# Alisah-Ozcan/HEonGPU

Hardware: AMD Instinct MI355X
Metric: homomorphic mults/sec (CKKS N=2^16, L=16) + NTT GB/s vs HBM roofline (higher is better)
Workload: dtype u64

## Files before the change

heongpu_amd/csrc/fpmod.cuh:

```cuda
#pragma once
#include "modarith.cuh"

namespace hegpu {

enum FpSiteKind {
    FPS_NONE = 0, FPS_FWD_COL = 1, FPS_FWD_COL_DECOMP = 2, FPS_FWD_ROW = 3, FPS_FWD_SINGLE = 4, FPS_KS_ROW = 5,
    FPS_KS_ROW_SPLIT = 6, FPS_INV = 7, FPS_TFHE_PREP = 8, FPS_TFHE_BR = 9, FPS_KINDS = 10
};
enum FpMetric { FPM_MUL_Y = 0, FPM_MUL_W = 1, FPM_MUL_T = 2, FPM_SUM = 3, FPM_RED_IN = 4, FPM_ABS = 5, FPM_COUNT = 6 };
#define FP_SITE(kind, sub) ((kind) * 8 + (sub))
#define FP_STAGE_PRODUCT 24
#define FP_STAGE_SUMS 25
#define FP_STAGE_INPUT 29
#define FP_STAGE_OUT 30
#define FP_STAGES 32

#ifdef HEGPU_FP_AUDIT_HEADER
#include HEGPU_FP_AUDIT_HEADER
#else
#define FP_AUDIT_FC_FIELDS
#define FP_AUDIT_INIT(c, site)
#define FP_STAGE(c, s)
#define FP_AUDIT_MUL(y, wx, wy, k, t, c)
#define FP_AUDIT_REDUCE(x, r, c)
#define FP_AUDIT_CANON(r, c)
#define FP_AUDIT_VAL(c, metric, v)
#define FP_AUDIT_FROM_U64(v)
#define FP_AUDIT_TO_U64(r)
#endif

struct FC {
    double q;
    double qi;
    FP_AUDIT_FC_FIELDS
};
__device__ __forceinline__ FC make_fc(u64 q, int site = FPS_NONE)
{
    FC c;
    c.q = (double) q;
    c.qi = 1.0 / c.q;
    FP_AUDIT_INIT(c, site);
    (void) site;
    return c;
}
__device__ __forceinline__ double as_f64(u64 v) { return __longlong_as_double((long long) v); }
__device__ __forceinline__ u64 as_bits(double v) { return (u64) __double_as_longlong(v); }
__device__ __forceinline__ double fp_from_u64(u64 v)
{
    FP_AUDIT_FROM_U64(v);
    return as_f64(v | 0x4330000000000000ull) - 4503599627370496.0;
}
__device__ __forceinline__ double fp_from_u32(u32 v) { return fp_from_u64((u64) v); }
__device__ __forceinline__ u64 fp_to_u64(double r)
{
    FP_AUDIT_TO_U64(r);
    return as_bits(r + 4503599627370496.0) & 0xFFFFFFFFFFFFFull;
}
__device__ __forceinline__ double fp_reduce(double x, const FC& c)
{
    const double r = __builtin_fma(-__builtin_rint(x * c.qi), c.q, x);
    FP_AUDIT_REDUCE(x, r, c);
    return r;
}
__device__ __forceinline__ double fp_canon(double x, const FC& c)
{
    const double r = fp_reduce(x, c);
    const double o = r < 0.0 ? r + c.q : r;
// ... 15 lines not shown
```

heongpu_amd/csrc/ntt.hip:

```cpp
#include "ntt.hpp"
#define HEGPU_FP_TU ntt
#include "fpmod.cuh"

namespace hegpu {

#define NTT_THREADS 256

#ifdef NTT_ABLATION_HEADER
#include NTT_ABLATION_HEADER
#else
__device__ __forceinline__ u64 gld(const u64* p) { return *p; }
__device__ __forceinline__ void gst(u64* p, u64 v) { *p = v; }
#define NTT_ABLATE_BFLY(x, y, w)
#define NTT_ABLATE_FPBFLY(x, y, w)
#define NTT_ABLATE_TW(load, root0, s) (load)
#define NTT_FP_TW(t, i, c) ((t)[i])
#endif

__device__ __forceinline__ u64 csub(u64 x, u64 m) { return (x >= m) ? x - m : x; }

typedef unsigned long long u64x2_t __attribute__((ext_vector_type(2)));
struct ConstTw {
    const u64x2_t __attribute__((address_space(4)))* p;
    __device__ __forceinline__ ulonglong2 operator[](u32 i) const
// ... 120 lines not shown
        const int half = 8 >> s;
        if (s > 0) __builtin_amdgcn_sched_barrier(0);
        if (s > 0) FP_STAGE(c, (c).stage + 1);
#pragma unroll
        for (int b = 0; b < (1 << s); b++) {
            const double wd = tb[((1 << s) - 1 + b) * 16];
            const ulonglong2 w = make_ulonglong2(as_bits(wd), as_bits(wd * c.qi));
#pragma unroll
            for (int j = 0; j < half; j++) fp_ct_bfly(x[b * 2 * half + j], x[b * 2 * half + j + half], w, c);
        }
    }
    FP_STAGE(c, (c).stage + 1);
#pragma unroll
    for (int k = 0; k < 16; k++) x[k] = fp_canon(x[k], c);
}

struct QC {
    u64 q;
    u64 q4;
    u32 nq0, nq1;
};
__device__ __forceinline__ QC make_qc(u64 q)
{
    QC c;
    c.q = q;
    c.q4 = 4 * q;
    u64 nq = 0 - q;
    c.nq0 = (u32) nq;
    c.nq1 = (u32) (nq >> 32);
    return c;
}

__device__ __forceinline__ u64 shoup_lazy(u64 y, ulonglong2 w, const QC& c)
{
    const u32 y0 = (u32) y, y1 = (u32) (y >> 32);
    const u32 w0 = (u32) w.x, w1 = (u32) (w.x >> 32), p0 = (u32) w.y, p1 = (u32) (w.y >> 32);
    const u64 A = (u64) y0 * p1;
    const u64 B = (u64) y1 * p0 + (u32) A;
    const u64 qh = (u64) y1 * p1 + (A >> 32) + (B >> 32);
    const u32 h0 = (u32) qh, h1 = (u32) (qh >> 32);
    u64 acc = (u64) y0 * w0;
    acc += (u64) h0 * c.nq0;
    const u32 hi = y0 * w1 + y1 * w0 + h0 * c.nq1 + h1 * c.nq0;
    return acc + ((u64) hi << 32);
}

__device__ __forceinline__ u64 shoup_full(u64 y, ulonglong2 w, const QC& c)
{
    u64 r = shoup_lazy(y, w, c);
    r = csub(r, 2 * c.q);
    return csub(r, c.q);
}

template <bool LAZY>
__device__ __forceinline__ void ct_bfly(u64& x, u64& y, ulonglong2 w, const QC& c)
{
    NTT_ABLATE_BFLY(x, y, w);
    u64 u = LAZY ? x : csub(x, c.q4);
    u64 t = shoup_lazy(y, w, c);
    x = u + t;
    y = u + c.q4 - t;
}

__device__ __forceinline__ void gs_bfly(u64& x, u64& y, ulonglong2 w, const QC& c)
{
    NTT_ABLATE_BFLY(x, y, w);
    u64 s = x + y;
    u64 d = x + c.q4 - y;
    x = csub(s, c.q4);
    y = shoup_lazy(d, w, c);
}

template <int LOGR, bool LAZY, typename TW>
__device__ __forceinline__ void ct_radix(u64 (&x)[1 << LOGR], TW tw,
                                         u32 root0, const QC& c)
{
#pragma unroll
    for (int s = 0; s < LOGR; s++) {
        const int half = (1 << LOGR) >> (s + 1);
#pragma unroll
        for (int b = 0; b < (1 << s); b++) {
            ulonglong2 w = NTT_ABLATE_TW(tw[(root0 << s) + b], root0, s);
#pragma unroll
            for (int j = 0; j < half; j++)
                ct_bfly<LAZY>(x[b * 2 * half + j], x[b * 2 * half + j + half], w, c);
        }
    }
}

template <bool LAZY>
__device__ __forceinline__ void ct_radix16_tb(u64 (&x)[16], const ulonglong2* __restrict__ tb, const QC& c)
{
#pragma unroll
    for (int s = 0; s < 4; s++) {
        const int half = 8 >> s;
#pragma unroll
        for (int b = 0; b < (1 << s); b++) {
            ulonglong2 w = tb[((1 << s) - 1 + b) * 16];
#pragma unroll
            for (int j = 0; j < half; j++)
                ct_bfly<LAZY>(x[b * 2 * half + j], x[b * 2 * half + j + half], w, c);
        }
    }
}

template <int LOGR>
__device__ __forceinline__ void gs_radix(u64 (&x)[1 << LOGR], const ulonglong2* __restrict__ tw,
                                         u32 root0, const QC& c)
{
#pragma unroll
    for (int s = LOGR - 1; s >= 0; s--) {
        const int half = (1 << LOGR) >> (s + 1);
#pragma unroll
        for (int b = 0; b < (1 << s); b++) {
            ulonglong2 w = NTT_ABLATE_TW(tw[(root0 << s) + b], root0, s);
#pragma unroll
            for (int j = 0; j < half; j++)
                gs_bfly(x[b * 2 * half + j], x[b * 2 * half + j + half], w, c);
        }
    }
}

__device__ __forceinline__ void gs_radix16_tb(u64 (&x)[16], const ulonglong2* __restrict__ tb, const QC& c)
{
#pragma unroll
    for (int s = 3; s >= 0; s--) {
        const int half = 8 >> s;
#pragma unroll
        for (int b = 0; b < (1 << s); b++) {
            ulonglong2 w = tb[((1 << s) - 1 + b) * 16];
#pragma unroll
            for (int j = 0; j < half; j++)
                gs_bfly(x[b * 2 * half + j], x[b * 2 * half + j + half], w, c);
        }
    }
}

template <int LOGR>
__device__ __forceinline__ void gs_radix_last(u64 (&x)[1 << LOGR], const ulonglong2* __restrict__ tw,
                                              u32 root0, ulonglong2 ninv, ulonglong2 w1ninv, const QC& c)
{
#pragma unroll
    for (int s = LOGR - 1; s >= 1; s--) {
        const int half = (1 << LOGR) >> (s + 1);
#pragma unroll
        for (int b = 0; b < (1 << s); b++) {
            ulonglong2 w = NTT_ABLATE_TW(tw[(root0 << s) + b], root0, s);
#pragma unroll
            for (int j = 0; j < half; j++)
                gs_bfly(x[b * 2 * half + j], x[b * 2 * half + j + half], w, c);
        }
    }
    const int half = (1 << LOGR) >> 1;
#pragma unroll
// ... 15 lines not shown
__device__ __forceinline__ int udiv16(int x, unsigned magic)
{
    return magic ? (int) __umulhi((unsigned) x, magic) : x;
}

__device__ __forceinline__ PolySel select_poly(const NttArgs& a, int poly)
{
    PolySel s;
    if (a.group_span) {
        const int k = udiv16(poly, a.mg_group_span), r = poly - k * a.group_span;
        if (a.polys_per_item) {
            const int per_item = udiv16(a.polys_per_item, a.mg_mod_count);
            const int it = udiv16(r, a.mg_per_item), d = r - it * per_item;
            poly = it * a.polys_per_item + d * a.mod_count + k;
        } else {
            poly = r * a.mod_count + k;
        }
    }
    int item = 0, j = poly;
    if (a.polys_per_item) {
        item = udiv16(poly, a.mg_polys_per_item);
        j = poly - item * a.polys_per_item;
    }
    int k = j - udiv16(j, a.mg_mod_count) * a.mod_count;
    if (a.mod_order) k = a.mod_order[k];
    s.mod = a.mod_offset + k;
    u64 slot = a.poly_order ? (u64) a.poly_order[j] : (u64) j;
    s.digit = a.decomp_mods ? udiv16(j, a.mg_decomp_mods) : -1;
    u64 in_slot = a.decomp_mods ? (u64) s.digit * (a.decomp_in_mul ? a.decomp_in_mul : 1) + a.decomp_in_add : slot;
    if (a.decomp_out_mul) slot = (u64) s.digit * a.decomp_out_mul + (u64) (j - s.digit * a.decomp_mods);
    s.in_off = (u64) item * a.in_item_stride + (in_slot << a.n_power);
    s.out_off = (u64) item * a.out_item_stride + (slot << a.n_power);
    s.item = item;
    s.j = j;
    return s;
}

__device__ __forceinline__ int col_phys(int e) { return e ^ (((e >> 8) & 1) << 4); }
__device__ __forceinline__ int row_phys(int e) { return e ^ (((e >> 5) & 7) << 1); }

__device__ __forceinline__ void wave_lds_fence()
{
    __builtin_amdgcn_fence(__ATOMIC_RELEASE, "wavefront");
    __builtin_amdgcn_wave_barrier();
    __builtin_amdgcn_fence(__ATOMIC_ACQUIRE, "wavefront");
}

#define COL_LDS_ELEMS 4096
#define ROW_LDS_ELEMS 4096

__device__ __forceinline__ bool fwd_stages_lazy(const Mod& md, u64 lazy_q_max) { return md.q <= lazy_q_max; }
#define NTT_ROW_LAZY_MAX_Q 0x0666666666666666ull
__device__ __forceinline__ bool row_stages_lazy(const Mod& md, u64 lazy_q_max) { return md.q <= lazy_q_max || md.q <= NTT_ROW_LAZY_MAX_Q; }

template <int S1, bool DECOMP, bool LAZY, bool SREG = false>
__device__ __forceinline__ void fwd_col_body(const NttArgs& a, const PolySel& ps, const Mod& md, u64* lds,
                                             const u64* sreg = nullptr)
{
    constexpr int R = 1 << S1;
    constexpr int CT = 4096 / R;
    constexpr int NSA = S1 - 4;
    constexpr int RA = 1 << NSA;
    constexpr int G = 16 / RA;
    const int t = threadIdx.x;
    const QC qc = make_qc(md.q);
    const ulonglong2* __restrict__ tw = a.tw + ((u64) ps.mod << a.n_power);
    const u64* __restrict__ src = a.in + ps.in_off + blockIdx.x * CT;
    u64* __restrict__ dst = a.out + ps.out_off + blockIdx.x * CT;

    const u64 half_qP = a.half_on ? a.mods[a.half_src_mod].q : 0;
    const u64 half_hm = a.half_on ? a.half_mod[ps.mod] : 0;
    u64 x[16];
    const int col = t % CT, r1 = t / CT;
    u64 v[16];
    if constexpr (NSA > 0) {
#pragma unroll
        for (int g = 0; g < G; g++) {
            const int L = t + NTT_THREADS * g;
            const int c = L % CT, rb = L / CT;
#pragma unroll
            for (int k = 0; k < RA; k++) v[g * RA + k] = SREG ? sreg[g * RA + k] : gld(&src[(u64) (rb + 16 * k) * 256 + c]);
        }
    } else {
#pragma unroll
        for (int k = 0; k < 16; k++) v[k] = SREG ? sreg[k] : gld(&src[(u64) k * 256 + col]);
    }
    if (DECOMP && a.half_on) {
#pragma unroll
        for (int k = 0; k < 16; k++) v[k] = sub_mod(reduce64(add_mod(v[k], a.half, half_qP), md), half_hm, md.q);
    } else if (DECOMP && !LAZY && a.mods[ps.digit].q > 8 * md.q) {
#pragma unroll
        for (int k = 0; k < 16; k++) v[k] = reduce64(v[k], md);
    }
    if constexpr (NSA > 0) {
#pragma unroll
        for (int g = 0; g < G; g++) {
            const int L = t + NTT_THREADS * g;
            const int c = L % CT, rb = L / CT;
            u64 y[RA];
#pragma unroll
            for (int k = 0; k < RA; k++) y[k] = v[g * RA + k];
            ct_radix<NSA, LAZY>(y, tw, 1u, qc);
#pragma unroll
            for (int k = 0; k < RA; k++) lds[col_phys((rb + 16 * k) * CT + c)] = y[k];
        }
        __syncthreads();
#pragma unroll
        for (int k = 0; k < 16; k++) x[k] = lds[col_phys((16 * r1 + k) * CT + col)];
        if (SREG) __syncthreads();
    } else {
#pragma unroll
        for (int k = 0; k < 16; k++) x[k] = v[k];
    }
    ct_radix<4, LAZY>(x, tw, (u32) (RA + r1), qc);
#pragma unroll
    for (int k = 0; k < 16; k++) gst(&dst[(u64) (16 * r1 + k) * 256 + col], x[k]);
}

template <int S1, bool DECOMP, bool WIDE, bool SREG = false>
__device__ __forceinline__ void fwd_col_body_fp(const NttArgs& a, const PolySel& ps, const Mod& md, u64* lds,
                                                ulonglong2* twl, const u64* sreg = nullptr)
{
    constexpr int R = 1 << S1;
    constexpr int CT = 4096 / R;
    constexpr int NSA = S1 - 4;
    constexpr int RA = 1 << NSA;
    constexpr int G = 16 / RA;
    const int t = threadIdx.x;
    const FC fc = make_fc(md.q, FP_SITE(DECOMP ? FPS_FWD_COL_DECOMP : FPS_FWD_COL, S1 - 4));
    const ulonglong2* __restrict__ tw = a.tw + ((u64) ps.mod << a.n_power);
    const u64* __restrict__ src = a.in + ps.in_off + blockIdx.x * CT;
    u64* __restrict__ dst = a.out + ps.out_off + blockIdx.x * CT;

    double c32 = 0.0, c32i = 0.0;
    if constexpr (DECOMP && WIDE) {
        c32 = (double) reduce64(1ull << 32, md);
        c32i = c32 * fc.qi;
    }
    const u64 half_qP = (DECOMP && a.half_on) ? a.mods[a.half_src_mod].q : 0;
    const double half_hm = (DECOMP && a.half_on) ? fp_from_u64(a.half_mod[ps.mod]) : 0.0;
    const bool in_small = S1 != 7 && DECOMP && !WIDE && !a.half_on && a.mods[ps.digit].q <= md.q + (md.q >> 6);
    typedef FpColSched<S1> CS;
    auto load_all = [&](auto& y, auto addr, int si0) {
        constexpr int CNT = sizeof(y) / sizeof(y[0]);
        FP_STAGE(fc, FP_STAGE_INPUT);
        if constexpr (SREG && !WIDE) {
            if (in_small) {
#pragma unroll
                for (int k = 0; k < CNT; k++) y[k] = as_f64(sreg[si0 + k]);
            } else {
#pragma unroll
                for (int k = 0; k < CNT; k++) y[k] = fp_reduce(as_f64(sreg[si0 + k]), fc);
            }
        } else {
            u64 v[CNT];
#pragma unroll
            for (int k = 0; k < CNT; k++) {
                v[k] = SREG ? sreg[si0 + k] : *addr(k);
                if constexpr (SREG) asm volatile("" : "+v"(v[k]));
            }
            if (!SREG && DECOMP && a.half_on) {
#pragma unroll
                for (int k = 0; k < CNT; k++) v[k] = add_mod(v[k], a.half, half_qP);
            }
#pragma unroll
            for (int k = 0; k < CNT; k++) {
                if constexpr (DECOMP && WIDE) y[k] = fp_mul(fp_from_u32((u32) (v[k] >> 32)), c32, c32i, fc) + fp_from_u32((u32) v[k]);
// ... 26 lines not shown
        }
        twl[t] = mine;
        __syncthreads();
#pragma unroll
        for (int k = 0; k < 16; k++) x[k] = as_f64(lds[col_phys((16 * r1 + k) * CT + col)]);
        if (SREG) __syncthreads();
        fp_ct_radix<4>(x, twl, (u32) (RA + r1), fc, CS::b_before, CS::b_at_end);
    } else {
        load_all(x, [&](int k) { return &src[(u64) k * 256 + col]; }, 0);
        fp_ct_radix<4>(x, tw, (u32) (RA + r1), fc, CS::b_before, CS::b_at_end);
    }
#pragma unroll
    for (int k = 0; k < 16; k++) {
        if constexpr (SREG) __builtin_nontemporal_store(as_bits(x[k]), &dst[(u64) (16 * r1 + k) * 256 + col]);
        else dst[(u64) (16 * r1 + k) * 256 + col] = as_bits(x[k]);
    }
}

template <int S1, bool DECOMP>
__global__ __launch_bounds__(NTT_THREADS) void ntt_fwd_col(NttArgs a)
{
    __shared__ u64 lds[(S1 > 4) ? COL_LDS_ELEMS : 1];
    __shared__ ulonglong2 twl[(S1 > 4) ? 256 : 1];
    int poly = blockIdx.y;
    if (DECOMP && a.only_int && a.int_slot_count > 0) {
        const int cnt = a.int_slot_count, digits = a.polys_per_item / a.decomp_mods;
        const int per_item = digits * cnt;
        const int item = poly / per_item, r = poly - item * per_item;
        const int digit = r / cnt, w = r - digit * cnt;
        poly = item * a.polys_per_item + digit * a.decomp_mods + a.int_slots[w];
    }
    const PolySel ps = select_poly(a, poly);
    if (DECOMP && a.skip_identity && ps.mod == ps.digit) return;
    const Mod md = a.mods[ps.mod];
    if (DECOMP && a.only_int && md.fp) return;
    if (DECOMP && a.copy_src) {
        constexpr int CT = 4096 >> S1;
        const int t = threadIdx.x, col = t % CT, r1 = t / CT;
        const u64 limb = ((u64) (ps.digit * a.copy_part_limbs + (ps.j - ps.digit * a.decomp_mods)) << a.n_power) +
                         blockIdx.x * CT;
        const u64* __restrict__ cs = a.copy_src + (u64) ps.item * a.copy_src_item_stride + limb;
        u64* __restrict__ cd = a.copy_dst + (u64) ps.item * a.copy_dst_item_stride + limb;
        u64 c[16];
#pragma unroll
        for (int k = 0; k < 16; k++) c[k] = cs[(u64) (16 * r1 + k) * 256 + col];
#pragma unroll
        for (int k = 0; k < 16; k++) cd[(u64) (16 * r1 + k) * 256 + col] = c[k];
    }
    if (md.fp) {
        if (DECOMP && a.mods[a.half_on ? a.half_src_mod : ps.digit].bit > 52)
            fwd_col_body_fp<S1, DECOMP, true>(a, ps, md, lds, twl);
        else fwd_col_body_fp<S1, DECOMP, false>(a, ps, md, lds, twl);
    } else if (fwd_stages_lazy(md, a.lazy_q_max)) fwd_col_body<S1, DECOMP, true>(a, ps, md, lds);
    else fwd_col_body<S1, DECOMP, false>(a, ps, md, lds);
}

__device__ __forceinline__ void row_store_all(const NttArgs& a, const PolySel& ps, const Mod& md, u64* __restrict__ p,
                                              u64 e0, const u64* lds, int row, int i0)
{
    if (!a.epi.on) {
#pragma unroll
        for (int k = 0; k < 16; k++) gst(&p[e0 + 16 * k], lds[row_phys(row * 256 + i0 + 16 * k)]);
        return;
    }
    const NttEpilogue& ep = a.epi;
    const int part = udiv16(ps.j, ep.mg_limbs), limb = ps.j - part * ep.limbs;
    const u64* __restrict__ ks = ep.ks + ep.ks_item_stride * ps.item + ((u64) (part * ep.ks_part_limbs + limb) << a.n_power) + e0;
    const u64 off = ((u64) (part * ep.limbs + limb) << a.n_power);
    const bool with_ct = ep.ct && (!ep.ct_parts || part < ep.ct_parts);
    const u64* ct = with_ct ? ep.ct + ep.ct_item_stride * ps.item + off + e0 : nullptr;
    u64* out = ep.out + ep.out_item_stride * ps.item + off;
    const u64 inv = ep.inv[ps.mod];
#pragma unroll
    for (int h = 0; h < 2; h++) {
        u64 kv[8], cv[8];
#pragma unroll
        for (int k = 0; k < 8; k++) kv[k] = ks[16 * (8 * h + k)];
        if (with_ct) {
#pragma unroll
            for (int k = 0; k < 8; k++) cv[k] = ct[16 * (8 * h + k)];
        }
        u64 r[8];
#pragma unroll
        for (int k = 0; k < 8; k++)
            r[k] = mul_barrett(sub_mod(kv[k], lds[row_phys(row * 256 + i0 + 16 * (8 * h + k))], md.q), inv, md);
        if (with_ct) {
#pragma unroll
            for (int k = 0; k < 8; k++) r[k] = add_mod(cv[k], r[k], md.q);
        }
        if (ep.galois_inv) {
#pragma unroll
            for (int k = 0; k < 8; k++) {
                const u32 e = (u32) e0 + 16 * (8 * h + k);
                const u32 ex = ((2u * (__brev(e) >> (32 - a.n_power)) + 1u) * ep.galois_inv) & ((2u << a.n_power) - 1u);
                out[__brev((ex - 1u) >> 1) >> (32 - a.n_power)] = r[k];
            }
        } else {
#pragma unroll
            for (int k = 0; k < 8; k++) out[e0 + 16 * (8 * h + k)] = r[k];
        }
    }
}

template <bool LAZY>
__device__ __forceinline__ void fwd_row_body(const NttArgs& a, const PolySel& ps, const Mod& md, u64* lds)
{
    const int t = threadIdx.x;
    const QC qc = make_qc(md.q);
    const int s1 = a.n_power - 8;
    const ulonglong2* __restrict__ tw = a.tw + ((u64) ps.mod << a.n_power);
    u64* __restrict__ p = a.out + ps.out_off + (u64) blockIdx.x * 4096;

    const int row = t >> 4, i0 = t & 15;
    const u32 crow = blockIdx.x * 16 + row;
    u64 x[16];
#pragma unroll
    for (int k = 0; k < 16; k++) x[k] = gld(&p[row * 256 + i0 + 16 * k]);
    ct_radix<4, LAZY>(x, tw, (1u << s1) + crow, qc);
#pragma unroll
    for (int k = 0; k < 16; k++) lds[row_phys(row * 256 + i0 + 16 * k)] = x[k];
    wave_lds_fence();
#pragma unroll
    for (int k = 0; k < 8; k++) {
        ulonglong2 v = *reinterpret_cast<const ulonglong2*>(&lds[row_phys(row * 256 + 16 * i0 + 2 * k)]);
        x[2 * k] = v.x;
        x[2 * k + 1] = v.y;
    }
    ct_radix16_tb<LAZY>(x, a.twB + ((u64) ps.mod * (15u << (a.n_power - 4))) + ((u64) crow * 15 * 16 + i0), qc);
    if (LAZY) {
#pragma unroll
        for (int k = 0; k < 16; k++) x[k] = reduce64(x[k], md);
    } else {
#pragma unroll
        for (int k = 0; k < 16; k++) x[k] = csub(csub(csub(x[k], qc.q4), 2 * qc.q), qc.q);
    }
    wave_lds_fence();
#pragma unroll
    for (int k = 0; k < 8; k++)
        *reinterpret_cast<ulonglong2*>(&lds[row_phys(row * 256 + 16 * i0 + 2 * k)]) =
            make_ulonglong2(x[2 * k], x[2 * k + 1]);
    wave_lds_fence();
    row_store_all(a, ps, md, a.out + ps.out_off, (u64) blockIdx.x * 4096 + row * 256 + i0, lds, row, i0);
}

__device__ __forceinline__ void fwd_row_body_fp(const NttArgs& a, const PolySel& ps, const Mod& md, u64* lds)
{
    const int t = threadIdx.x;
    const FC fc = make_fc(md.q, FP_SITE(FPS_FWD_ROW, a.n_power - 12));
    const int s1 = a.n_power - 8;
    const ulonglong2* __restrict__ tw = a.tw + ((u64) ps.mod << a.n_power);
    u64* __restrict__ p = a.out + ps.out_off + (u64) blockIdx.x * 4096;

    const int row = t >> 4, i0 = t & 15;
    const u32 crow = blockIdx.x * 16 + row;
    double x[16];
#pragma unroll
    for (int k = 0; k < 16; k++) x[k] = as_f64(p[row * 256 + i0 + 16 * k]);
    fp_ct_radix<4>(x, tw, (1u << s1) + crow, fc, 0u, true);
#pragma unroll
    for (int k = 0; k < 16; k++) lds[row_phys(row * 256 + i0 + 16 * k)] = as_bits(x[k]);
    wave_lds_fence();
#pragma unroll
    for (int k = 0; k < 8; k++) {
        ulonglong2 v = *reinterpret_cast<const ulonglong2*>(&lds[row_phys(row * 256 + 16 * i0 + 2 * k)]);
        x[2 * k] = as_f64(v.x);
        x[2 * k + 1] = as_f64(v.y);
    }
    fp_ct_radix16_tb8(x, a.twB8 + ((u64) ps.mod * (15u << (a.n_power - 4))) + ((u64) crow * 15 * 16 + i0), fc);
    wave_lds_fence();
#pragma unroll
    for (int k = 0; k < 8; k++)
        *reinterpret_cast<ulonglong2*>(&lds[row_phys(row * 256 + 16 * i0 + 2 * k)]) =
            make_ulonglong2(fp_to_u64(x[2 * k]), fp_to_u64(x[2 * k + 1]));
    wave_lds_fence();
    row_store_all(a, ps, md, a.out + ps.out_off, (u64) blockIdx.x * 4096 + row * 256 + i0, lds, row, i0);
}

__global__ __launch_bounds__(NTT_THREADS) void ntt_fwd_row(NttArgs a)
{
    __shared__ __attribute__((aligned(16))) u64 lds[ROW_LDS_ELEMS];
    const PolySel ps = select_poly(a, blockIdx.y);
    if (a.skip_identity && ps.mod == ps.digit) return;
    const Mod md = a.mods[ps.mod];
    if (md.fp) fwd_row_body_fp(a, ps, md, lds);
    else if (row_stages_lazy(md, a.lazy_q_max)) fwd_row_body<true>(a, ps, md, lds);
    else fwd_row_body<false>(a, ps, md, lds);
}

template <int S1>
__device__ __forceinline__ int single_pos(int row, int col)
{
    return (row >> 4) * 4096 + row_phys((row & 15) * 256 + col);
}

template <int S1, bool FP, bool LAZY, bool DECOMP = false>
__device__ __forceinline__ void fwd_single_body(const NttArgs& a, const PolySel& ps, const Mod& md, u64* limb)
{
    constexpr int R = 1 << S1;
    constexpr int CT = 4096 / R;
    constexpr int NSA = S1 - 4;
    constexpr int RA = 1 << NSA;
    constexpr int G = 16 / RA;
    const int t = threadIdx.x, g = t >> 8, tt = t & 255;
    const QC qc = make_qc(md.q);
    const FC fc = make_fc(md.q, FP_SITE(FPS_FWD_SINGLE, S1 - 4));
    const ulonglong2* __restrict__ tw = a.tw + ((u64) ps.mod << a.n_power);
    const u64* __restrict__ src = a.in + ps.in_off + g * CT;
    const int col = tt % CT, r1 = tt / CT;
    u64 dv[DECOMP ? 16 : 1];
    double dy[(DECOMP && FP) ? 16 : 1];
    if constexpr (DECOMP) {
        if constexpr (NSA > 0) {
#pragma unroll
            for (int gi = 0; gi < G; gi++) {
                const int L = tt + 256 * gi;
                const int c = L % CT, rb = L / CT;
#pragma unroll
                for (int k = 0; k < RA; k++) dv[gi * RA + k] = src[(u64) (rb + 16 * k) * 256 + c];
            }
        } else {
#pragma unroll
            for (int k = 0; k < 16; k++) dv[k] = src[(u64) k * 256 + col];
        }
        const u64 half_qP = a.half_on ? a.mods[a.half_src_mod].q : 0;
        if constexpr (FP) {
            FP_STAGE(fc, FP_STAGE_INPUT);
            if (a.half_on) {
#pragma unroll
                for (int k = 0; k < 16; k++) dv[k] = add_mod(dv[k], a.half, half_qP);
            }
            if (a.mods[a.half_on ? a.half_src_mod : ps.digit].bit > 52) {
                const double c32 = (double) reduce64(1ull << 32, md), c32i = c32 * fc.qi;
#pragma unroll
                for (int k = 0; k < 16; k++)
                    dy[k] = fp_mul(fp_from_u32((u32) (dv[k] >> 32)), c32, c32i, fc) + fp_from_u32((u32) dv[k]);
            } else {
#pragma unroll
                for (int k = 0; k < 16; k++) dy[k] = fp_reduce(fp_from_u64(dv[k]), fc);
// ... 101 lines not shown
#pragma unroll
        for (int k = 0; k < 16; k++) r[k] = fp_to_u64(x[k]);
    } else {
        u64 x[16];
#pragma unroll
        for (int k = 0; k < 16; k++) x[k] = lds[row_phys(row * 256 + i0 + 16 * k)];
        ct_radix<4, LAZY>(x, tw, (1u << S1) + crow, qc);
#pragma unroll
        for (int k = 0; k < 16; k++) lds[row_phys(row * 256 + i0 + 16 * k)] = x[k];
        wave_lds_fence();
#pragma unroll
        for (int k = 0; k < 8; k++) {
            ulonglong2 v = *reinterpret_cast<const ulonglong2*>(&lds[row_phys(row * 256 + 16 * i0 + 2 * k)]);
            x[2 * k] = v.x;
            x[2 * k + 1] = v.y;
        }
        ct_radix16_tb<LAZY>(x, tb, qc);
        if (LAZY) {
#pragma unroll
            for (int k = 0; k < 16; k++) r[k] = reduce64(x[k], md);
        } else {
#pragma unroll
            for (int k = 0; k < 16; k++) r[k] = csub(csub(csub(x[k], qc.q4), 2 * qc.q), qc.q);
        }
    }
    wave_lds_fence();
#pragma unroll
    for (int k = 0; k < 8; k++)
        *reinterpret_cast<ulonglong2*>(&lds[row_phys(row * 256 + 16 * i0 + 2 * k)]) = make_ulonglong2(r[2 * k], r[2 * k + 1]);
    wave_lds_fence();
    row_store_all(a, ps, md, a.out + ps.out_off, (u64) g * 4096 + row * 256 + i0, lds, row, i0);
}

template <int S1, bool DECOMP = false>
__global__ __launch_bounds__(16 << S1, 4) void ntt_fwd_single(NttArgs a)
{
    extern __shared__ __attribute__((aligned(16))) u64 limb[];
    const PolySel ps = select_poly(a, blockIdx.x);
    if (DECOMP && a.skip_identity && ps.mod == ps.digit) return;
    const Mod md = a.mods[ps.mod];
    if (md.fp) fwd_single_body<S1, true, false, DECOMP>(a, ps, md, limb);
    else if (fwd_stages_lazy(md, a.lazy_q_max)) fwd_single_body<S1, false, true, DECOMP>(a, ps, md, limb);
    else fwd_single_body<S1, false, false, DECOMP>(a, ps, md, limb);
}

__device__ __forceinline__ void acc128(u64& hi, u64& lo, u64 a, u64 b)
{
    u64 h, l;
    mul64wide(a, b, h, l);
    lo += l;
    hi += h + (lo < l);
}

template <bool LAZY>
__device__ __forceinline__ void ks_row_digit(u64 (&x)[16], const u64* __restrict__ p, u64* lds,
                                             const ulonglong2* twa, const ulonglong2* __restrict__ tb,
                                             const QC& qc, const Mod& md, int row, int i0)
{
#pragma unroll
    for (int k = 0; k < 16; k++) x[k] = gld(&p[row * 256 + i0 + 16 * k]);
#pragma unroll
    for (int s = 0; s < 4; s++) {
        const int half = 8 >> s;
#pragma unroll
        for (int b = 0; b < (1 << s); b++) {
            const ulonglong2 w = twa[((1 << s) - 1 + b) * 16 + row];
#pragma unroll
            for (int j = 0; j < half; j++) ct_bfly<LAZY>(x[b * 2 * half + j], x[b * 2 * half + j + half], w, qc);
        }
    }
#pragma unroll
    for (int k = 0; k < 16; k++) lds[row_phys(row * 256 + i0 + 16 * k)] = x[k];
    wave_lds_fence();
#pragma unroll
    for (int k = 0; k < 8; k++) {
        ulonglong2 v = *reinterpret_cast<const ulonglong2*>(&lds[row_phys(row * 256 + 16 * i0 + 2 * k)]);
        x[2 * k] = v.x;
        x[2 * k + 1] = v.y;
    }
    ct_radix16_tb<LAZY>(x, tb, qc);
    if (!LAZY) {
#pragma unroll
        for (int k = 0; k < 16; k++) x[k] = csub(csub(csub(x[k], qc.q4), 2 * qc.q), qc.q);
    }
    wave_lds_fence();
#pragma unroll
    for (int k = 0; k < 8; k++)
        *reinterpret_cast<ulonglong2*>(&lds[row_phys(row * 256 + 16 * i0 + 2 * k)]) =
            make_ulonglong2(x[2 * k], x[2 * k + 1]);
    wave_lds_fence();
#pragma unroll
    for (int k = 0; k < 16; k++) x[k] = lds[row_phys(row * 256 + i0 + 16 * k)];
    wave_lds_fence();
}

struct KsIdx { int item, tile, slot; bool valid; int d0, d1; };
__host__ __device__ __forceinline__ unsigned ks_slots(const KsMacArgs& a, int kind)
{
    const int all = a.slot_count ? a.slot_count : a.rc;
    if (a.int_slot_count <= 0 || kind == 0) return (unsigned) all;
    return kind == 1 ? (unsigned) a.int_slot_count : (unsigned) (all - a.int_slot_count);
}
template <bool SPLIT, int KIND = 0>
__device__ __forceinline__ KsIdx ks_index(const KsMacArgs& a)
{
    const unsigned b = blockIdx.x, xcd = b & 7u, j = b >> 3;
    const unsigned splits = SPLIT ? (unsigned) a.splits : 1u;
    const unsigned units = (unsigned) a.items * splits;
    const unsigned tiles = 1u << (a.n_power - 12);
    const unsigned total = ks_slots(a, KIND) * tiles * units, chunk = (total + 7u) >> 3;
    const unsigned lin = xcd * chunk + j;
    const unsigned g = lin / units, unit = lin - g * units;
    const unsigned item = SPLIT ? unit / splits : unit, sp = SPLIT ? unit - item * splits : 0u;
    const unsigned nslots = ks_slots(a, KIND), gt = g / nslots;
    KsIdx r;
    r.valid = lin < total;
    r.item = (int) item;
    r.tile = (int) gt;
    int si = (int) (g - gt * nslots);
    if (KIND == 1 && a.int_slot_count > 0) {
        si = a.int_slots[r.valid ? si : 0];
    } else {
        si += a.slot_first;
        if (KIND == 2 && a.int_slot_count > 0) {
#pragma unroll
            for (int q = 0; q < 8; q++)
                if (q < a.int_slot_count && a.int_slots[q] <= si) si++;
        }
    }
    r.slot = si;
    r.d0 = SPLIT ? (int) (sp * (unsigned) a.digits / splits) : 0;
    r.d1 = SPLIT ? (int) ((sp + 1) * (unsigned) a.digits / splits) : a.digits;
    return r;
}

__device__ __forceinline__ void ks_tail_store(const KsMacArgs& a, int item, int slot, int p, u64 e0, const Mod& md, u64 inv,
                                              const u64 (&acc)[16], const u64 (&tv)[16], bool with_ct, const u64 (&cv)[16])
{
    const KsMacArgs::Tail& e = a.tail;
    u64* out = e.out + e.out_item_stride * item + ((u64) (p * e.limbs + slot) << a.n_power);
    u64 r[16];
#pragma unroll
    for (int k = 0; k < 16; k++) r[k] = mul_barrett(sub_mod(acc[k], tv[k], md.q), inv, md);
    if (with_ct) {
#pragma unroll
        for (int k = 0; k < 16; k++) r[k] = add_mod(cv[k], r[k], md.q);
    }
    if (e.galois_inv) {
#pragma unroll
        for (int k = 0; k < 16; k++) {
            const u32 el = (u32) e0 + 16 * k;
            const u32 ex = ((2u * (__brev(el) >> (32 - a.n_power)) + 1u) * e.galois_inv) & ((2u << a.n_power) - 1u);
            out[__brev((ex - 1u) >> 1) >> (32 - a.n_power)] = r[k];
        }
    } else {
#pragma unroll
        for (int k = 0; k < 16; k++) out[e0 + 16 * k] = r[k];
    }
}
__device__ __forceinline__ const u64* ks_tail_T(const KsMacArgs& a, int item, int slot, int tile, int p)
{
    return a.tail.T + a.tail.T_item_stride * item + ((u64) (p * a.rc + slot) << a.n_power) + (u64) tile * 4096;
}
__device__ __forceinline__ bool ks_tail_ct(const KsMacArgs& a, int item, int slot, int p, u64 e0, u64 (&cv)[16])
{
    const KsMacArgs::Tail& e = a.tail;
    if (!e.ct || (e.ct_parts && p >= e.ct_parts)) return false;
    const u64* c = e.ct + e.ct_item_stride * item + ((u64) (p * e.limbs + slot) << a.n_power) + e0;
#pragma unroll
    for (int k = 0; k < 16; k++) cv[k] = c[16 * k];
    return true;
}

#define KS_TW_LDS_BYTES ((15 * 256 + 15 * 16) * 8)
template <bool SPLIT, bool MD = false>
__device__ __forceinline__ void ks_row_mac_int_body(const KsMacArgs& a, const KsIdx& ki, const Mod& md, int midx,
                                                    u64* lds, void* twbuf)
{
    const int t = threadIdx.x;
    const int item = ki.item, tile = ki.tile, slot = ki.slot;
    const QC qc = make_qc(md.q);
    const int s1 = a.n_power - 8;
    const ulonglong2* __restrict__ tw = a.tw + ((u64) midx << a.n_power);
    const int row = t >> 4, i0 = t & 15;
    const u32 crow = tile * 16 + row;
    const ulonglong2* __restrict__ tb = a.twB + ((u64) midx * (15u << (a.n_power - 4))) + ((u64) crow * 15 * 16 + i0);
    const u64 n = (u64) 1 << a.n_power;
    const u64* __restrict__ pin = a.in + a.in_item_stride * item + ((u64) slot << a.n_power) + (u64) tile * 4096;
    const u64* __restrict__ pk = a.key + ((u64) midx << a.n_power) + (u64) tile * 4096 + row * 256 + i0;
    const u64 dig_off = (u64) a.rc << a.n_power;
    const u64 key_off1 = (u64) a.key_limbs << a.n_power, key_off2 = (u64) a.key_limbs << (a.n_power + 1);
    const bool lazy = row_stages_lazy(md, a.lazy_q_max) && md.q <= ~0ull / (u64) a.digits;
    ulonglong2* twa = reinterpret_cast<ulonglong2*>(twbuf);
    if (i0 < 15) {
        const int s = (i0 >= 7) ? 3 : (i0 >= 3) ? 2 : (i0 >= 1) ? 1 : 0;
        twa[i0 * 16 + row] = tw[((((u32) 1 << s1) + crow) << s) + (i0 - ((1 << s) - 1))];
    }
    wave_lds_fence();

    const int item_s = MD ? __builtin_amdgcn_readfirstlane(item) : 0, slot_s = MD ? __builtin_amdgcn_readfirstlane(slot) : 0;
    const int tile_s = MD ? __builtin_amdgcn_readfirstlane(tile) : 0, midx_s = MD ? __builtin_amdgcn_readfirstlane(midx) : 0;
    u64 h0[16], l0[16], h1[16], l1[16];
#pragma unroll
    for (int k = 0; k < 16; k++) h0[k] = l0[k] = h1[k] = l1[k] = 0;
    for (int i = ki.d0; i < ki.d1; i++) {
        u64 x[16];
        const u64* p = pin + dig_off * i;
        if (a.skip_identity && i == midx) {
            const u64* pi = a.ident + a.ident_item_stride * item + ((u64) i << a.n_power) + (u64) tile * 4096;
#pragma unroll
            for (int k = 0; k < 16; k++) x[k] = gld(&pi[row * 256 + i0 + 16 * k]);
        } else if (lazy) {
            ks_row_digit<true>(x, p, lds, twa, tb, qc, md, row, i0);
        } else {
            ks_row_digit<false>(x, p, lds, twa, tb, qc, md, row, i0);
        }
        const u64* k0 = pk + key_off2 * i;
        const u64* k1 = k0 + key_off1;
#pragma unroll
        for (int k = 0; k < 16; k++) {
            acc128(h0[k], l0[k], x[k], k0[16 * k]);
            acc128(h1[k], l1[k], x[k], k1[16 * k]);
        }
    }
    if constexpr (MD) {
        u64 acc0[16], acc1[16];
#pragma unroll
        for (int k = 0; k < 16; k++) {
            acc0[k] = reduce128(h0[k], l0[k], md);
            acc1[k] = reduce128(h1[k], l1[k], md);
        }
        int tt = threadIdx.x;
        asm volatile("" : "+v"(tt));
        const int trow = tt >> 4, ti0 = tt & 15;
        const u64 e0 = (u64) tile_s * 4096 + trow * 256 + ti0;
        const u64 inv = a.tail.inv[midx_s];
        const bool lazy_t = row_stages_lazy(md, a.lazy_q_max);
        const ulonglong2* __restrict__ ttb = a.twB + ((u64) midx_s * (15u << (a.n_power - 4))) + ((u64) (tile_s * 16 + trow) * 15 * 16 + ti0);
        auto part = [&](int p, const u64 (&acc)[16]) {
            u64 cv[16], x[16];
            const bool with_ct = ks_tail_ct(a, item_s, slot_s, p, e0, cv);
            const u64* pT = ks_tail_T(a, item_s, slot_s, tile_s, p);
            if (lazy_t) {
                ks_row_digit<true>(x, pT, lds, twa, ttb, qc, md, trow, ti0);
#pragma unroll
                for (int k = 0; k < 16; k++) x[k] = reduce64(x[k], md);
            } else {
                ks_row_digit<false>(x, pT, lds, twa, ttb, qc, md, trow, ti0);
            }
            ks_tail_store(a, item_s, slot_s, p, e0, md, inv, acc, x, with_ct, cv);
        };
        __builtin_amdgcn_sched_barrier(0);
        part(0, acc0);
        __builtin_amdgcn_sched_barrier(0);
        part(1, acc1);
        return;
    }
    u64* po = (SPLIT ? const_cast<u64*>(pin) + dig_off * ki.d0 - (u64) tile * 4096
                     : a.out + a.out_item_stride * item + ((u64) slot << a.n_power)) +
              (u64) tile * 4096 + row * 256 + i0;
#pragma unroll
    for (int k = 0; k < 16; k++) {
        po[16 * k] = reduce128(h0[k], l0[k], md);
        po[dig_off + 16 * k] = reduce128(h1[k], l1[k], md);
    }
    (void) n;
}

template <bool SPLIT>
__global__ __launch_bounds__(NTT_THREADS, SPLIT ? 2 : 1) void ks_row_mac(KsMacArgs a)
{
    __shared__ __attribute__((aligned(16))) u64 lds[ROW_LDS_ELEMS];
    __shared__ ulonglong2 twa[15 * 16];
    const KsIdx ki = ks_index<SPLIT, SPLIT ? 0 : 1>(a);
    if (!ki.valid) return;
    const int midx = a.mod_order ? a.mod_order[ki.slot] : ki.slot;
    const Mod md = a.mods[midx];
    if (md.fp) return;
    ks_row_mac_int_body<SPLIT>(a, ki, md, midx, lds, twa);
}

template <bool SPLIT>
__device__ __forceinline__ void ks_fp_row(double (&x)[16], const u64 (&xr)[16], const double* twl, u64* lds, const FC& fc,
                                          int s1, int row, int i0, int t)
{
    if constexpr (SPLIT) {
#pragma unroll
        for (int k = 0; k < 16; k++) x[k] = as_f64(xr[k]);
#pragma unroll
        for (int s = 0; s < 4; s++) {
            const int half = 8 >> s;
            FP_STAGE(fc, s1 + s);
#pragma unroll
            for (int b = 0; b < (1 << s); b++) {
                const double w = twl[15 * 256 + ((1 << s) - 1 + b) * 16 + row];
                const ulonglong2 wp = make_ulonglong2(as_bits(w), as_bits(w * fc.qi));
#pragma unroll
                for (int j = 0; j < half; j++) fp_ct_bfly(x[b * 2 * half + j], x[b * 2 * half + j + half], wp, fc);
            }
// ... 136 lines not shown
    for (int k = 0; k < 16; k++) a0[k] = a1[k] = 0.0;
    int since = 0;
    for (int i = ki.d0; i < ki.d1; i++) {
        double x[16];
        const u64* p = pin + dig_off * i;
        const bool ident = a.skip_identity && i == midx;
        const u64* px = ident ? a.ident + a.ident_item_stride * item + ((u64) i << a.n_power) + (u64) tile * 4096 : p;
        u64 xr[16];
#pragma unroll
        for (int k = 0; k < 16; k++) {
            if constexpr (!SPLIT) xr[k] = __builtin_nontemporal_load(&px[row * 256 + i0 + 16 * k]);
            else xr[k] = px[row * 256 + i0 + 16 * k];
        }
        const u64* k0 = pk + key_off2 * i;
        const u64* k1 = k0 + key_off1;
        u64 kv0[16], kv1[16];
#pragma unroll
        for (int k = 0; k < 16; k++) {
            kv0[k] = k0[16 * k];
            kv1[k] = k1[16 * k];
        }
        if (ident) {
            FP_STAGE(fc, FP_STAGE_INPUT);
#pragma unroll
            for (int k = 0; k < 16; k++) x[k] = fp_reduce(fp_from_u64(xr[k]), fc);
        } else {
            ks_fp_row<SPLIT>(x, xr, twl, lds, fc, s1, row, i0, t);
        }
#pragma unroll
        for (int k = 0; k < 16; k++) {
            const double xi = x[k] * fc.qi;
            FP_STAGE(fc, FP_STAGE_PRODUCT);
            a0[k] += fp_mul(fp_from_u64(kv0[k]), x[k], xi, fc);
            a1[k] += fp_mul(fp_from_u64(kv1[k]), x[k], xi, fc);
            FP_STAGE(fc, FP_STAGE_SUMS + since);
            FP_AUDIT_VAL(fc, FPM_SUM, a0[k]);
            FP_AUDIT_VAL(fc, FPM_SUM, a1[k]);
        }
        if (++since == 3) {
            since = 0;
            FP_STAGE(fc, FP_STAGE_SUMS + 3);
#pragma unroll
            for (int k = 0; k < 16; k++) {
                a0[k] = fp_reduce(a0[k], fc);
                a1[k] = fp_reduce(a1[k], fc);
            }
        }
    }
    if constexpr (MD) {
        int tt = threadIdx.x;
        asm volatile("" : "+v"(tt));
        const int trow = tt >> 4, ti0 = tt & 15;
        const u64 e0 = (u64) tile_s * 4096 + trow * 256 + ti0;
        const Mod mds = a.mods[midx_s];
        const u64 inv = a.tail.inv[midx_s];
        auto part = [&](int p, const double (&acc)[16]) {
            const u64* pT = ks_tail_T(a, item_s, slot_s, tile_s, p);
            u64 tr[16], cv[16];
#pragma unroll
            for (int k = 0; k < 16; k++) tr[k] = __builtin_nontemporal_load(&pT[trow * 256 + ti0 + 16 * k]);
            const bool with_ct = ks_tail_ct(a, item_s, slot_s, p, e0, cv);
            double x[16];
            ks_fp_row<false>(x, tr, twl, lds, fc, s1, trow, ti0, tt);
            FP_STAGE(fc, FP_STAGE_OUT);
            u64 av[16], tv[16];
#pragma unroll
            for (int k = 0; k < 16; k++) {
                av[k] = fp_to_u64(fp_canon(acc[k], fc));
                tv[k] = fp_to_u64(fp_canon(x[k], fc));
            }
            ks_tail_store(a, item_s, slot_s, p, e0, mds, inv, av, tv, with_ct, cv);
        };
        __builtin_amdgcn_sched_barrier(0);
        part(0, a0);
        __builtin_amdgcn_sched_barrier(0);
        part(1, a1);
        return;
    }
    u64* po = (SPLIT ? const_cast<u64*>(pin) + dig_off * ki.d0 - (u64) tile * 4096
                     : a.out + a.out_item_stride * item + ((u64) slot << a.n_power)) +
              (u64) tile * 4096 + row * 256 + i0;
    FP_STAGE(fc, FP_STAGE_OUT);
#pragma unroll
    for (int k = 0; k < 16; k++) {
        if constexpr (!SPLIT) {
            __builtin_nontemporal_store(fp_to_u64(fp_canon(a0[k], fc)), &po[16 * k]);
            __builtin_nontemporal_store(fp_to_u64(fp_canon(a1[k], fc)), &po[dig_off + 16 * k]);
        } else {
            po[16 * k] = fp_to_u64(fp_canon(a0[k], fc));
            po[dig_off + 16 * k] = fp_to_u64(fp_canon(a1[k], fc));
        }
    }
}

template <bool SPLIT>
__global__ __launch_bounds__(NTT_THREADS) void ks_row_mac_fp(KsMacArgs a)
{
    __shared__ __attribute__((aligned(16))) u64 lds[ROW_LDS_ELEMS];
    __shared__ double twl[15 * 256 + 15 * 16];
    const KsIdx ki = ks_index<SPLIT, SPLIT ? 0 : 2>(a);
    if (!ki.valid) return;
    const int midx = a.mod_order ? a.mod_order[ki.slot] : ki.slot;
    const Mod md = a.mods[midx];
    if (!md.fp) return;
    ks_row_mac_fp_body<SPLIT>(a, ki, md, midx, lds, twl);
}

__global__ __launch_bounds__(NTT_THREADS) void ks_row_mac_fp_moddown(KsMacArgs a)
{
    __shared__ __attribute__((aligned(16))) u64 lds[ROW_LDS_ELEMS];
    __shared__ double twl[15 * 256 + 15 * 16];
    const KsIdx ki = ks_index<false, 2>(a);
    if (!ki.valid) return;
    const int midx = a.mod_order ? a.mod_order[ki.slot] : ki.slot;
    const Mod md = a.mods[midx];
    if (!md.fp) return;
    ks_row_mac_fp_body<false, true>(a, ki, md, midx, lds, twl);
}
__global__ __launch_bounds__(NTT_THREADS, 1) void ks_row_mac_moddown(KsMacArgs a)
{
    __shared__ __attribute__((aligned(16))) u64 lds[ROW_LDS_ELEMS];
    __shared__ ulonglong2 twa[15 * 16];
    const KsIdx ki = ks_index<false, 1>(a);
    if (!ki.valid) return;
// ... 788 lines not shown
```

Baseline: 8349.

## Schedule lazy NTT corrections by modulus headroom and keep keyswitch tail in floating point

Adds a compile-time correction schedule for Cooley-Tukey butterflies that, for moduli of 60 bits or less, performs conditional subtractions only in the stages where value growth would overflow, instead of in every stage. This is applied to the non-lazy forward column, row and keyswitch row paths. Separately, the FP64 keyswitch tail now does the subtract, multiply-by-inverse and add in double arithmetic before a single canonicalisation, rather than converting both operands to integers and using Barrett reduction. The intent is to cut integer compare/subtract and 64-bit multiply work, at the cost of more template instantiations and tighter bounds reasoning.

```diff
diff --git a/heongpu_amd/csrc/fpmod.cuh b/heongpu_amd/csrc/fpmod.cuh
--- a/heongpu_amd/csrc/fpmod.cuh
+++ b/heongpu_amd/csrc/fpmod.cuh
@@ -13,6 +13,7 @@
 #define FP_STAGE_SUMS 25
 #define FP_STAGE_INPUT 29
 #define FP_STAGE_OUT 30
+#define FP_STAGE_TAIL 31
 #define FP_STAGES 32
 
 #ifdef HEGPU_FP_AUDIT_HEADER
diff --git a/heongpu_amd/csrc/ntt.hip b/heongpu_amd/csrc/ntt.hip
--- a/heongpu_amd/csrc/ntt.hip
+++ b/heongpu_amd/csrc/ntt.hip
@@ -196,15 +196,39 @@
     return csub(r, c.q);
 }
 
-template <bool LAZY>
-__device__ __forceinline__ void ct_bfly(u64& x, u64& y, ulonglong2 w, const QC& c)
+struct CsSched { unsigned c8, c4; };
+__host__ __device__ constexpr CsSched cs_sched(int stages, int room)
+{
+    CsSched r{0u, 0u};
+    int b = 8;
+    for (int s = 0; s < stages; s++) {
+        const int need = (s == stages - 1) ? 4 : room - 4;
+        if (b > need && b > 8) {
+            r.c8 |= 1u << s;
+            b = 8;
+        }
+        if (b > need) {
+            r.c4 |= 1u << s;
+            b = 4;
+        }
+        b += 4;
+    }
+    return r;
+}
+static_assert(cs_sched(8, 8).c8 == 0u && cs_sched(8, 8).c4 == 0xFFu, "61-bit moduli: a correction in every stage");
+static_assert(cs_sched(8, 16).c8 == 0xD4u && cs_sched(8, 16).c4 == 0x80u, "60-bit moduli: stages 2, 4, 6, 7 / 7");
+static_assert(cs_sched(5, 16).c8 == 0x14u && cs_sched(5, 16).c4 == 0x10u, "N = 2^13 column pass: stages 2, 4 / 4");
+__device__ __forceinline__ void ct_bfly_cs(u64& x, u64& y, ulonglong2 w, const QC& c, int cs)
 {
     NTT_ABLATE_BFLY(x, y, w);
-    u64 u = LAZY ? x : csub(x, c.q4);
+    u64 u = x;
+    if (cs & 2) u = csub(u, 2 * c.q4);
+    if (cs & 1) u = csub(u, c.q4);
     u64 t = shoup_lazy(y, w, c);
     x = u + t;
     y = u + c.q4 - t;
 }
+#define NTT_CS_EVERY 0xFFFFFFFFu
 
 __device__ __forceinline__ void gs_bfly(u64& x, u64& y, ulonglong2 w, const QC& c)
 {
@@ -215,35 +239,37 @@
     y = shoup_lazy(d, w, c);
 }
 
-template <int LOGR, bool LAZY, typename TW>
+template <int LOGR, bool LAZY, unsigned C8 = 0u, unsigned C4 = NTT_CS_EVERY, typename TW>
 __device__ __forceinline__ void ct_radix(u64 (&x)[1 << LOGR], TW tw,
                                          u32 root0, const QC& c)
 {
 #pragma unroll
     for (int s = 0; s < LOGR; s++) {
         const int half = (1 << LOGR) >> (s + 1);
+        const int cs = LAZY ? 0 : (int) (((C8 >> s) & 1u) * 2u + ((C4 >> s) & 1u));
 #pragma unroll
         for (int b = 0; b < (1 << s); b++) {
             ulonglong2 w = NTT_ABLATE_TW(tw[(root0 << s) + b], root0, s);
 #pragma unroll
             for (int j = 0; j < half; j++)
-                ct_bfly<LAZY>(x[b * 2 * half + j], x[b * 2 * half + j + half], w, c);
-        }
-    }
-}
-
-template <bool LAZY>
+                ct_bfly_cs(x[b * 2 * half + j], x[b * 2 * half + j + half], w, c, cs);
+        }
+    }
+}
+
+template <bool LAZY, unsigned C8 = 0u, unsigned C4 = NTT_CS_EVERY>
 __device__ __forceinline__ void ct_radix16_tb(u64 (&x)[16], const ulonglong2* __restrict__ tb, const QC& c)
 {
 #pragma unroll
     for (int s = 0; s < 4; s++) {
         const int half = 8 >> s;
+        const int cs = LAZY ? 0 : (int) (((C8 >> s) & 1u) * 2u + ((C4 >> s) & 1u));
 #pragma unroll
         for (int b = 0; b < (1 << s); b++) {
             ulonglong2 w = tb[((1 << s) - 1 + b) * 16];
 #pragma unroll
             for (int j = 0; j < half; j++)
-                ct_bfly<LAZY>(x[b * 2 * half + j], x[b * 2 * half + j + half], w, c);
+                ct_bfly_cs(x[b * 2 * half + j], x[b * 2 * half + j + half], w, c, cs);
         }
     }
 }
@@ -365,11 +391,13 @@
 __device__ __forceinline__ bool fwd_stages_lazy(const Mod& md, u64 lazy_q_max) { return md.q <= lazy_q_max; }
 #define NTT_ROW_LAZY_MAX_Q 0x0666666666666666ull
 __device__ __forceinline__ bool row_stages_lazy(const Mod& md, u64 lazy_q_max) { return md.q <= lazy_q_max || md.q <= NTT_ROW_LAZY_MAX_Q; }
-
-template <int S1, bool DECOMP, bool LAZY, bool SREG = false>
+__device__ __forceinline__ bool stages_room16(const Mod& md) { return md.bit <= 60; }
+
+template <int S1, bool DECOMP, bool LAZY, bool SREG = false, int ROOM = 8>
 __device__ __forceinline__ void fwd_col_body(const NttArgs& a, const PolySel& ps, const Mod& md, u64* lds,
                                              const u64* sreg = nullptr)
 {
+    constexpr CsSched CS = cs_sched(S1, ROOM);
     constexpr int R = 1 << S1;
     constexpr int CT = 4096 / R;
     constexpr int NSA = S1 - 4;
@@ -413,7 +441,7 @@
             u64 y[RA];
 #pragma unroll
             for (int k = 0; k < RA; k++) y[k] = v[g * RA + k];
-            ct_radix<NSA, LAZY>(y, tw, 1u, qc);
+            ct_radix<NSA, LAZY, CS.c8, CS.c4>(y, tw, 1u, qc);
 #pragma unroll
             for (int k = 0; k < RA; k++) lds[col_phys((rb + 16 * k) * CT + c)] = y[k];
         }
@@ -425,7 +453,7 @@
 #pragma unroll
         for (int k = 0; k < 16; k++) x[k] = v[k];
     }
-    ct_radix<4, LAZY>(x, tw, (u32) (RA + r1), qc);
+    ct_radix<4, LAZY, (CS.c8 >> NSA), (CS.c4 >> NSA)>(x, tw, (u32) (RA + r1), qc);
 #pragma unroll
     for (int k = 0; k < 16; k++) gst(&dst[(u64) (16 * r1 + k) * 256 + col], x[k]);
 }
@@ -558,6 +586,7 @@
             fwd_col_body_fp<S1, DECOMP, true>(a, ps, md, lds, twl);
         else fwd_col_body_fp<S1, DECOMP, false>(a, ps, md, lds, twl);
     } else if (fwd_stages_lazy(md, a.lazy_q_max)) fwd_col_body<S1, DECOMP, true>(a, ps, md, lds);
+    else if (S1 > 4 && stages_room16(md)) fwd_col_body<S1, DECOMP, false, false, (S1 > 4 ? 16 : 8)>(a, ps, md, lds);
     else fwd_col_body<S1, DECOMP, false>(a, ps, md, lds);
 }
 
@@ -608,9 +637,10 @@
     }
 }
 
-template <bool LAZY>
+template <bool LAZY, int ROOM = 8>
 __device__ __forceinline__ void fwd_row_body(const NttArgs& a, const PolySel& ps, const Mod& md, u64* lds)
 {
+    constexpr CsSched CS = cs_sched(8, ROOM);
     const int t = threadIdx.x;
     const QC qc = make_qc(md.q);
     const int s1 = a.n_power - 8;
@@ -622,7 +652,7 @@
     u64 x[16];
 #pragma unroll
     for (int k = 0; k < 16; k++) x[k] = gld(&p[row * 256 + i0 + 16 * k]);
-    ct_radix<4, LAZY>(x, tw, (1u << s1) + crow, qc);
+    ct_radix<4, LAZY, CS.c8, CS.c4>(x, tw, (1u << s1) + crow, qc);
 #pragma unroll
     for (int k = 0; k < 16; k++) lds[row_phys(row * 256 + i0 + 16 * k)] = x[k];
     wave_lds_fence();
@@ -632,7 +662,7 @@
         x[2 * k] = v.x;
         x[2 * k + 1] = v.y;
     }
-    ct_radix16_tb<LAZY>(x, a.twB + ((u64) ps.mod * (15u << (a.n_power - 4))) + ((u64) crow * 15 * 16 + i0), qc);
+    ct_radix16_tb<LAZY, (CS.c8 >> 4), (CS.c4 >> 4)>(x, a.twB + ((u64) ps.mod * (15u << (a.n_power - 4))) + ((u64) crow * 15 * 16 + i0), qc);
     if (LAZY) {
 #pragma unroll
         for (int k = 0; k < 16; k++) x[k] = reduce64(x[k], md);
@@ -690,6 +720,7 @@
     const Mod md = a.mods[ps.mod];
     if (md.fp) fwd_row_body_fp(a, ps, md, lds);
     else if (row_stages_lazy(md, a.lazy_q_max)) fwd_row_body<true>(a, ps, md, lds);
+    else if (stages_room16(md)) fwd_row_body<false, 16>(a, ps, md, lds);
     else fwd_row_body<false>(a, ps, md, lds);
 }
 
@@ -897,21 +928,23 @@
     hi += h + (lo < l);
 }
 
-template <bool LAZY>
+template <bool LAZY, int ROOM = 8>
 __device__ __forceinline__ void ks_row_digit(u64 (&x)[16], const u64* __restrict__ p, u64* lds,
                                              const ulonglong2* twa, const ulonglong2* __restrict__ tb,
                                              const QC& qc, const Mod& md, int row, int i0)
 {
+    constexpr CsSched CS = cs_sched(8, ROOM);
 #pragma unroll
     for (int k = 0; k < 16; k++) x[k] = gld(&p[row * 256 + i0 + 16 * k]);
 #pragma unroll
     for (int s = 0; s < 4; s++) {
         const int half = 8 >> s;
+        const int cs = LAZY ? 0 : (int) (((CS.c8 >> s) & 1u) * 2u + ((CS.c4 >> s) & 1u));
 #pragma unroll
         for (int b = 0; b < (1 << s); b++) {
             const ulonglong2 w = twa[((1 << s) - 1 + b) * 16 + row];
 #pragma unroll
-            for (int j = 0; j < half; j++) ct_bfly<LAZY>(x[b * 2 * half + j], x[b * 2 * half + j + half], w, qc);
+            for (int j = 0; j < half; j++) ct_bfly_cs(x[b * 2 * half + j], x[b * 2 * half + j + half], w, qc, cs);
         }
     }
 #pragma unroll
@@ -923,7 +956,7 @@
         x[2 * k] = v.x;
         x[2 * k + 1] = v.y;
     }
-    ct_radix16_tb<LAZY>(x, tb, qc);
+    ct_radix16_tb<LAZY, (CS.c8 >> 4), (CS.c4 >> 4)>(x, tb, qc);
     if (!LAZY) {
 #pragma unroll
         for (int k = 0; k < 16; k++) x[k] = csub(csub(csub(x[k], qc.q4), 2 * qc.q), qc.q);
@@ -979,18 +1012,10 @@
     return r;
 }
 
-__device__ __forceinline__ void ks_tail_store(const KsMacArgs& a, int item, int slot, int p, u64 e0, const Mod& md, u64 inv,
-                                              const u64 (&acc)[16], const u64 (&tv)[16], bool with_ct, const u64 (&cv)[16])
+__device__ __forceinline__ void ks_tail_scatter(const KsMacArgs& a, int item, int slot, int p, u64 e0, const u64 (&r)[16])
 {
     const KsMacArgs::Tail& e = a.tail;
     u64* out = e.out + e.out_item_stride * item + ((u64) (p * e.limbs + slot) << a.n_power);
-    u64 r[16];
-#pragma unroll
-    for (int k = 0; k < 16; k++) r[k] = mul_barrett(sub_mod(acc[k], tv[k], md.q), inv, md);
-    if (with_ct) {
-#pragma unroll
-        for (int k = 0; k < 16; k++) r[k] = add_mod(cv[k], r[k], md.q);
-    }
     if (e.galois_inv) {
 #pragma unroll
         for (int k = 0; k < 16; k++) {
@@ -1002,6 +1027,41 @@
 #pragma unroll
         for (int k = 0; k < 16; k++) out[e0 + 16 * k] = r[k];
     }
+}
+__device__ __forceinline__ void ks_tail_store(const KsMacArgs& a, int item, int slot, int p, u64 e0, const Mod& md, u64 inv,
+                                              const u64 (&acc)[16], const u64 (&tv)[16], bool with_ct, const u64 (&cv)[16])
+{
+    u64 r[16];
+#pragma unroll
+    for (int k = 0; k < 16; k++) r[k] = mul_barrett(sub_mod(acc[k], tv[k], md.q), inv, md);
+    if (with_ct) {
+#pragma unroll
+        for (int k = 0; k < 16; k++) r[k] = add_mod(cv[k], r[k], md.q);
+    }
+    ks_tail_scatter(a, item, slot, p, e0, r);
+}
+__device__ __forceinline__ void ks_tail_store_fp(const KsMacArgs& a, int item, int slot, int p, u64 e0, const FC& fc, double inv,
+                                                 double invq, const double (&acc)[16], const double (&tv)[16], bool with_ct,
+                                                 const u64 (&cv)[16])
+{
+    double m[16];
+#pragma unroll
+    for (int k = 0; k < 16; k++) {
+        FP_STAGE(fc, FP_STAGE_OUT);
+        const double d = fp_reduce(acc[k], fc) - tv[k];
+        FP_STAGE(fc, FP_STAGE_TAIL);
+        FP_AUDIT_VAL(fc, FPM_SUM, d);
+        m[k] = fp_mul(d, inv, invq, fc);
+    }
+    FP_STAGE(fc, FP_STAGE_OUT);
+    if (with_ct) {
+#pragma unroll
+        for (int k = 0; k < 16; k++) m[k] += fp_from_u64(cv[k]);
+    }
+    u64 r[16];
+#pragma unroll
+    for (int k = 0; k < 16; k++) r[k] = fp_to_u64(fp_canon(m[k], fc));
+    ks_tail_scatter(a, item, slot, p, e0, r);
 }
 __device__ __forceinline__ const u64* ks_tail_T(const KsMacArgs& a, int item, int slot, int tile, int p)
 {
@@ -1036,6 +1096,7 @@
     const u64 dig_off = (u64) a.rc << a.n_power;
     const u64 key_off1 = (u64) a.key_limbs << a.n_power, key_off2 = (u64) a.key_limbs << (a.n_power + 1);
     const bool lazy = row_stages_lazy(md, a.lazy_q_max) && md.q <= ~0ull / (u64) a.digits;
+    const bool room16 = stages_room16(md);
     ulonglong2* twa = reinterpret_cast<ulonglong2*>(twbuf);
     if (i0 < 15) {
         const int s = (i0 >= 7) ? 3 : (i0 >= 3) ? 2 : (i0 >= 1) ? 1 : 0;
@@ -1057,6 +1118,8 @@
             for (int k = 0; k < 16; k++) x[k] = gld(&pi[row * 256 + i0 + 16 * k]);
         } else if (lazy) {
             ks_row_digit<true>(x, p, lds, twa, tb, qc, md, row, i0);
+        } else if (room16) {
+            ks_row_digit<false, 16>(x, p, lds, twa, tb, qc, md, row, i0);
         } else {
             ks_row_digit<false>(x, p, lds, twa, tb, qc, md, row, i0);
         }
@@ -1090,6 +1153,8 @@
                 ks_row_digit<true>(x, pT, lds, twa, ttb, qc, md, trow, ti0);
 #pragma unroll
                 for (int k = 0; k < 16; k++) x[k] = reduce64(x[k], md);
+            } else if (room16) {
+                ks_row_digit<false, 16>(x, pT, lds, twa, ttb, qc, md, trow, ti0);
             } else {
                 ks_row_digit<false>(x, pT, lds, twa, ttb, qc, md, trow, ti0);
             }
@@ -1332,8 +1397,7 @@
         asm volatile("" : "+v"(tt));
         const int trow = tt >> 4, ti0 = tt & 15;
         const u64 e0 = (u64) tile_s * 4096 + trow * 256 + ti0;
-        const Mod mds = a.mods[midx_s];
-        const u64 inv = a.tail.inv[midx_s];
+        const double inv = fp_from_u64(a.tail.inv[midx_s]), invq = inv * fc.qi;
         auto part = [&](int p, const double (&acc)[16]) {
             const u64* pT = ks_tail_T(a, item_s, slot_s, tile_s, p);
             u64 tr[16], cv[16];
@@ -1342,14 +1406,7 @@
             const bool with_ct = ks_tail_ct(a, item_s, slot_s, p, e0, cv);
             double x[16];
             ks_fp_row<false>(x, tr, twl, lds, fc, s1, trow, ti0, tt);
-            FP_STAGE(fc, FP_STAGE_OUT);
-            u64 av[16], tv[16];
-#pragma unroll
-            for (int k = 0; k < 16; k++) {
-                av[k] = fp_to_u64(fp_canon(acc[k], fc));
-                tv[k] = fp_to_u64(fp_canon(x[k], fc));
-            }
-            ks_tail_store(a, item_s, slot_s, p, e0, mds, inv, av, tv, with_ct, cv);
+            ks_tail_store_fp(a, item_s, slot_s, p, e0, fc, inv, invq, acc, x, with_ct, cv);
         };
         __builtin_amdgcn_sched_barrier(0);
         part(0, a0);
```

New measurement: 8509, median of 6. 1.02x the previous value.
